# LiWentomng/OrientedRepPoints

Hardware: AMD Instinct MI355X
Metric: images/sec (1024x1024 DOTA, R-50 FPN) (higher is better)
Workload: dtype f32; 1 GPU; configs[1]: OrientedRepPoints R-50 FPN inference, 1024x1024 patch, 15 classes, bs=1/GPU, nms_pre=2000, score_thr=0.05, rnms iou_thr=0.4, max_per_img=2000; random-init weights, head biases calibrated to ~2000 dets/img; global_batch=1, parallelism=replicas x1 (image-parallel, no collective), images_in_flight_per_gpu=4

## Files before the change

include/orp_hip.h:

```cpp
#ifndef ORP_HIP_H_
#define ORP_HIP_H_

#include <stddef.h>
#include <stdint.h>

#ifdef __cplusplus
extern "C" {
#endif

#define ORP_OK 0
#define ORP_EINVAL (-1)
#define ORP_EWORKSPACE (-2)
#define ORP_ETOOBIG (-3)

const char* orp_version(void);

#define ORP_NMS_MAX_BOXES 131072
size_t orp_rnms_workspace_bytes(int n);
int orp_rnms(const float* dets, int n, float iou_thr, int flavor, int presorted, int order_out,
             int64_t* keep_out, int32_t* num_keep, void* workspace, size_t workspace_bytes, void* stream);

size_t orp_rnms_batched_workspace_bytes(int n_total, int nseg, int max_seg);
int orp_rnms_batched(const float* dets, int n_total, const int32_t* seg_offsets, int nseg, int max_seg,
                     float iou_thr, int flavor, int64_t* keep_out, int32_t* num_keep,
// ... 225 lines not shown
size_t orp_fpn_topdown_workspace_bytes(const orp_norm_level* levels, int nlevels, int batch, int channels, int groups);
int orp_fpn_topdown_nhwc(const orp_norm_level* levels, const float* const* gammas_host, const float* const* betas_host,
                         int nlevels, int batch, int channels, int groups, float eps, uint32_t* amax_out, void* workspace,
                         size_t workspace_bytes, void* stream);

typedef struct { const float* input; const float* residual; float* output; float* output2; int height; int width; } orp_bias_level;
int orp_bias_act_multi(const orp_bias_level* levels_host, int nlevels, int batch, int channels, const float* bias,
                       const float* sub, int relu, void* stream);

size_t orp_conv1x1_packed_floats(int c_in);
int orp_conv1x1_ok(int c_in, int c_out);
int orp_conv1x1_pack_weight(const float* weight, int c_out, int c_in, float* packed, void* stream);
int orp_conv1x1_multi(const orp_bias_level* levels_host, int nlevels, int batch, int c_in, int c_out,
                      const float* weight_packed, const float* bias, const float* sub, int relu, void* stream);

int orp_conv1x1_bn_act_ok(int c_in, int c_out);
int orp_conv1x1_bn_act_pays(int c_in, int c_out, int hw, int batch, int has_residual);
int orp_conv1x1_bn_act_tile(int c_in, int c_out, int hw, int batch, int* tile_channels, int* tile_positions);
int orp_conv1x1_bn_act(const float* x, const float* weight_t, const float* scale, const float* shift, const float* residual,
                       const float* scale2, const float* shift2, float* y, int batch, int c_in, int c_out, int hw, int relu,
                       void* stream);

int orp_conv1x1_bn_act_range(const float* x, const float* weight_t, const float* scale, const float* shift, const float* residual,
                             const float* scale2, const float* shift2, float* y, int batch, int c_in, int c_out, int hw, int relu,
                             uint32_t* range_out, void* stream);
int orp_conv1x1_bn_act_pieces_ok(int c_in, int c_out);
int orp_conv1x1_bn_act_pieces_pays(int c_in, int c_out, int hw, int batch, int has_residual);
int orp_conv1x1_bn_act_pieces_tile(int c_in, int c_out, int hw, int batch, int* tile_channels, int* tile_positions);
size_t orp_conv1x1_bn_pieces_packed_bytes(int c_in, int c_out);
int orp_conv1x1_bn_pieces_pack_weight(const float* weight, int c_in, int c_out, void* packed, void* stream);
int orp_conv1x1_bn_act_pieces(const float* x, const void* weight_packed, const float* scale, const float* shift,
                              const float* residual, const float* scale2, const float* shift2, float* y, int batch, int c_in,
                              int c_out, int hw, int relu, uint32_t* range_out, void* stream);

int orp_conv1x1_bn_act_pieces_dual_ok(int c_in, int c_in2, int c_out);
int orp_conv1x1_bn_act_pieces_dual_pays(int c_in, int c_in2, int c_out, int hw, int stride2, int batch);
int orp_conv1x1_bn_act_pieces_dual_tile(int c_in, int c_in2, int c_out, int hw, int batch, int* tile_channels, int* tile_positions);
int orp_conv1x1_bn_act_pieces_dual(const float* x, const void* w_packed, const float* scale, const float* shift, const float* x2,
                                   const void* w2_packed, const float* scale2, const float* shift2, int c_in2, int h2, int w2,
                                   int stride2, float* y, int batch, int c_in, int c_out, int ho, int wo, int relu, void* stream);

int orp_affine_act_range(const float* x, const float* residual, const float* scale, const float* shift, float* y, int batch,
                         int channels, int hw, int relu, uint32_t* range_out, void* stream);

int orp_conv3x3_bn_act_ok(int c_in, int c_out);
int orp_conv3x3_bn_act_pays(int c_in, int c_out, int height, int width, int batch);
int orp_conv3x3_bn_act_tile(int c_in, int c_out, int height, int width, int batch, int* tile_h, int* tile_w, int* waves_pos,
                            int* waves_ch);
size_t orp_conv3x3_bn_packed_bytes(int c_in, int c_out);
int orp_conv3x3_bn_pack_weight(const float* weight, int c_in, int c_out, void* packed, void* stream);
int orp_conv3x3_bn_act(const float* x, const void* weight_packed, const float* scale, const float* shift, const uint32_t* range_in,
                       float* y, int batch, int c_in, int c_out, int height, int width, int relu, void* stream);


int orp_conv3x3_small_ok(int c_in, int c_out);
int orp_conv3x3_small_multi(const orp_norm_level* levels_host, int nlevels, int batch, int c_in, int c_out,
                            const float* weight_packed, void* stream);
int orp_conv3x3_small_multi_ex(const orp_norm_level* levels_host, const float* const* weights_packed_host, int nlevels,
                               int batch, int c_in, int c_out, void* stream);
size_t orp_conv3x3_small_workspace_bytes(const orp_norm_level* levels_host, const int* strides_host, int nlevels, int batch,
                                         int c_out);
int orp_conv3x3_small_multi_strided(const orp_norm_level* levels_host, const float* const* weights_packed_host,
                                    const int* strides_host, int nlevels, int batch, int c_in, int c_out, void* workspace,
                                    size_t workspace_bytes, void* stream);

typedef struct { const float* input_a; const float* input_b; float* output_a; float* output_b; int height; int width; } orp_conv_level;
int orp_conv_split_ok(int c_in, int c_out, int kh, int kw);
int orp_conv_split_multi(const orp_conv_level* levels_host, int nlevels, int batch, int c_in, int c_out,
                         const float* weight_a_packed, const float* weight_b_packed, const float* bias_a, const float* bias_b,
                         int relu, int kh, int kw, int stride_h, int stride_w, int pad_h, int pad_w, int dil_h, int dil_w,
                         int out_layout, int nprod, void* workspace, size_t workspace_bytes, const uint32_t* amax_in,
                         int amax_stride, void* stream);
int orp_conv_split_multi_ex(const orp_conv_level* levels_host, const float* const* weights_packed_host,
                            const float* const* biases_host, int nlevels, int batch, int c_in, int c_out, int relu, int kh, int kw,
                            int stride_h, int stride_w, int pad_h, int pad_w, int dil_h, int dil_w, int out_layout, int nprod,
                            void* workspace, size_t workspace_bytes, const uint32_t* amax_in, void* stream);
size_t orp_conv_split_gn_partial_floats(const orp_conv_level* levels_host, int nlevels, int batch, int groups, int nlayers);
int orp_conv_split_multi_gn(const orp_conv_level* levels_host, int nlevels, int batch, int c_in, int c_out,
                            const float* weight_a_packed, const float* weight_b_packed, int kh, int kw, int pad_h, int pad_w,
                            int dil_h, int dil_w, int nprod, const float* coef_in, int relu_in, float* partials,
                            size_t partial_floats, int groups, void* workspace, size_t workspace_bytes, const uint32_t* amax_in,
                            int amax_stride, int amax_count, void* stream);
int orp_conv_split_gn_finish(const orp_conv_level* levels_host, int nlevels, int batch, int channels, int groups, int nlayers,
                             float eps, const float* const* gammas_host, const float* const* betas_host, const float* partials,
                             float* coef_out, uint32_t* bound_out, void* stream);
int orp_affine_act_multi_cl(const orp_norm_level* levels, int nlevels, int batch, int channels, const float* coef, int relu,
                            const uint32_t* bound_in, int nsets, int per_set, uint32_t* slot_out, void* stream);
int orp_conv_split_set_halo(int on);
int orp_conv_split_halo_tile(const orp_conv_level* levels_host, int nlevels, int batch, int c_in, int c_out, int kh, int kw, int stride,
                             int pad, int dil, int nprod, int* th, int* tw);
int orp_nchw_to_nhwc_multi(const orp_norm_level* levels_host, int nlevels, int batch, int channels, void* stream);
int orp_nchw_to_nhwc_multi_amax(const orp_norm_level* levels_host, int nlevels, int batch, int channels, const int* slots_host,
                                uint32_t* amax_out, int nslots, int reset, void* stream);

typedef struct { const float* input; const float* grad_output; int height; int width; } orp_wgrad_level;
int orp_conv_wgrad_split_ok(int c_in, int c_out, int kh, int kw);
size_t orp_conv_wgrad_split_workspace_bytes(const orp_wgrad_level* levels_host, int nlevels, int batch, int kh, int kw);
int orp_conv_wgrad_split(const orp_wgrad_level* levels_host, int nlevels, int batch, int c_in, int c_out, int kh, int kw,
                         int pad_h, int pad_w, int dil_h, int dil_w, const uint32_t* amax_x, const uint32_t* amax_g,
                         float* grad_weight, void* workspace, size_t workspace_bytes, void* stream);

int orp_window_attention(const float* qkv, const float* qkv_bias, const float* bias_table, int batch, int height, int width,
                         int heads, int head_dim, int window, int shift, float scale, float* out, void* stream);

int orp_window_attention_train(const float* qkv, const float* qkv_bias, const float* bias_table, int batch, int height, int width,
                               int heads, int head_dim, int window, int shift, float scale, float* out, float* lse, void* stream);
// ... 48 lines not shown
```

orientedreppoints_amd/_lib.py:

```python
import ctypes
import os

import torch

_HERE = os.path.dirname(os.path.abspath(__file__))
LIB_PATH = os.environ.get("ORP_HIP_LIB") or os.path.join(_HERE, "csrc", "liborp_hip.so")

ORP_OK, ORP_EINVAL, ORP_EWORKSPACE, ORP_ETOOBIG = 0, -1, -2, -3
ORP_NMS_MAX_BOXES = 131072

_vp = ctypes.c_void_p
_i = ctypes.c_int
_f = ctypes.c_float
_sz = ctypes.c_size_t

_SIGNATURES = {
    "orp_version": (ctypes.c_char_p, []),
    "orp_rnms_workspace_bytes": (_sz, [_i]),
    "orp_rnms": (_i, [_vp, _i, _f, _i, _i, _i, _vp, _vp, _vp, _sz, _vp]),
    "orp_rnms_batched_workspace_bytes": (_sz, [_i, _i, _i]),
    "orp_rnms_batched": (_i, [_vp, _i, _vp, _i, _i, _f, _i, _vp, _vp, _vp, _sz, _vp]),
    "_poly_nms": (None, [_vp, _vp, _vp, _i, _i, _f, _i]),
    "_overlaps": (None, [_vp, _vp, _vp, _i, _i, _i]),
    "orp_quad_iou_matrix": (_i, [_vp, _i, _vp, _i, _i, _i, _vp, _vp]),
# ... 43 lines not shown
    "orp_dcn_forward_h_tile_rows": (_i, [ctypes.c_long, _i]),
    "orp_dcn_forward_h_wave_specialised": (_i, []),
    "orp_dcn_forward_h_workspace_bytes": (_sz, [_vp, _i, _i, _i, _i]),
    "orp_dcn_forward_multi_h": (_i, [_vp, _vp, _i, _i, _i, _i, _vp, _vp] + [_i] * 12 + [_vp, _sz, _vp]),
    "orp_dcn_im2col": (_i, [_vp, _vp, _vp] + [_i] * 13 + [_vp, _vp]),
    "orp_dcn_col2im": (_i, [_vp, _vp, _vp, _vp] + [_i] * 13 + [_vp, _vp, _vp, _vp]),
    "orp_dcn_im2col_f64": (_i, [_vp, _vp, _vp] + [_i] * 13 + [_vp, _vp]),
    "orp_dcn_col2im_f64": (_i, [_vp, _vp, _vp, _vp] + [_i] * 13 + [_vp, _vp, _vp, _vp]),
    "orp_dcn_col2im_nhwc": (_i, [_vp, _vp, _vp] + [_i] * 12 + [_vp, _vp, _vp]),
    "orp_dcn_forward_direct": (_i, [_vp] * 6 + [_i] * 15 + [_vp]),
    "orp_dcn_backward_mfma_ok": (_i, [_i] * 6),
    "orp_dcn_backward_workspace_bytes": (_sz, [_vp] + [_i] * 10),
    "orp_dcn_backward_multi": (_i, [_vp, _i, _i, _i, _i, _vp, _vp] + [_i] * 9 + [_vp, _sz, _vp]),
    "orp_dcn_backward_multi_ex": (_i, [_vp, _vp, _vp, _i, _i, _i, _i, _i, _vp, _vp] + [_i] * 9 + [_vp, _sz, _vp]),
    "orp_poly_nms_f64_workspace_bytes": (_sz, [_i]),
    "orp_poly_nms_f64": (_i, [_vp, _i, ctypes.c_double, _vp, _vp, _vp, _sz, _vp]),
    "orp_poly_nms_f64_batched_workspace_bytes": (_sz, [_i, _i, _i]),
    "orp_poly_nms_f64_batched": (_i, [_vp, _i, _vp, _i, _i, ctypes.c_double, _i, _i, _vp, _vp, _vp, _sz, _vp]),
    "orp_scene_tiles": (_i, [_vp, _i, _i, ctypes.c_longlong, _vp, _i, _i, _vp, _vp, _i, _i, _vp, _vp]),
    "orp_scene_tiles_resized": (_i, [_vp, _i, _i, ctypes.c_longlong, _vp, _i, _i, _i, _i, _i, _i, _i, _vp, _vp, _vp, _vp, _vp, _vp, _i,
                                     _i, _vp, _vp]),
    "orp_scene_tiles_flip": (_i, [_vp, _i, _i, ctypes.c_longlong, _vp, _i, _i, _vp, _vp, _i, _i, _vp, _vp]),
    "orp_scene_tiles_resized_flip": (_i, [_vp, _i, _i, ctypes.c_longlong, _vp, _i, _i, _i, _i, _i, _i, _i, _vp, _vp, _vp, _vp, _vp,
                                          _vp, _i, _i, _vp, _vp]),
    "orp_scene_collect_workspace_bytes": (_sz, [_i, _i]),
    "orp_scene_collect": (_i, [_vp, _i, _i, _vp, ctypes.c_double, _i, _i, _vp, _vp, _vp, _vp, _vp, _sz, _vp]),
    "orp_soft_rnms_host": (_i, [_vp, _i, _f, _i, _f, _f, _vp, _vp]),
    "orp_conv1x1_packed_floats": (_sz, [_i]),
    "orp_conv1x1_ok": (_i, [_i, _i]),
    "orp_conv1x1_pack_weight": (_i, [_vp, _i, _i, _vp, _vp]),
    "orp_conv1x1_multi": (_i, [_vp, _i, _i, _i, _i, _vp, _vp, _vp, _i, _vp]),
    "orp_conv1x1_bn_act_ok": (_i, [_i, _i]),
    "orp_conv1x1_bn_act_pays": (_i, [_i, _i, _i, _i, _i]),
    "orp_conv1x1_bn_act_tile": (_i, [_i, _i, _i, _i, _vp, _vp]),
    "orp_conv1x1_bn_act": (_i, [_vp, _vp, _vp, _vp, _vp, _vp, _vp, _vp, _i, _i, _i, _i, _i, _vp]),
    "orp_conv1x1_bn_act_range": (_i, [_vp, _vp, _vp, _vp, _vp, _vp, _vp, _vp, _i, _i, _i, _i, _i, _vp, _vp]),
    "orp_affine_act_range": (_i, [_vp, _vp, _vp, _vp, _vp, _i, _i, _i, _i, _vp, _vp]),
    "orp_conv1x1_bn_act_pieces_ok": (_i, [_i, _i]),
    "orp_conv1x1_bn_act_pieces_pays": (_i, [_i, _i, _i, _i, _i]),
    "orp_conv1x1_bn_act_pieces_tile": (_i, [_i, _i, _i, _i, _vp, _vp]),
    "orp_conv1x1_bn_pieces_packed_bytes": (_sz, [_i, _i]),
    "orp_conv1x1_bn_pieces_pack_weight": (_i, [_vp, _i, _i, _vp, _vp]),
    "orp_conv1x1_bn_act_pieces": (_i, [_vp, _vp, _vp, _vp, _vp, _vp, _vp, _vp, _i, _i, _i, _i, _i, _vp, _vp]),
    "orp_conv1x1_bn_act_pieces_dual_ok": (_i, [_i, _i, _i]),
    "orp_conv1x1_bn_act_pieces_dual_pays": (_i, [_i, _i, _i, _i, _i, _i]),
    "orp_conv1x1_bn_act_pieces_dual_tile": (_i, [_i, _i, _i, _i, _i, _vp, _vp]),
    "orp_conv1x1_bn_act_pieces_dual": (_i, [_vp, _vp, _vp, _vp, _vp, _vp, _vp, _vp, _i, _i, _i, _i, _vp, _i, _i, _i, _i, _i, _i, _vp]),
    "orp_conv3x3_bn_act_ok": (_i, [_i, _i]),
    "orp_conv3x3_bn_act_pays": (_i, [_i, _i, _i, _i, _i]),
    "orp_conv3x3_bn_act_tile": (_i, [_i, _i, _i, _i, _i, _vp, _vp, _vp, _vp]),
    "orp_conv3x3_bn_packed_bytes": (_sz, [_i, _i]),
    "orp_conv3x3_bn_pack_weight": (_i, [_vp, _i, _i, _vp, _vp]),
    "orp_conv3x3_bn_act": (_i, [_vp, _vp, _vp, _vp, _vp, _vp, _i, _i, _i, _i, _i, _i, _vp]),
    "orp_pp_select_scratch_bytes": (_sz, [_i, _i, _i]),
    "orp_pp_select": (_i, [_vp, _i, _i, _vp, _i, _i, _vp, _vp, _sz, _vp]),
    "orp_pp_gather": (_i, [_vp, _vp, _i, _i, _vp, _vp, _vp, _i, _vp, _vp, _vp, _vp, _vp]),
    "orp_pp_compact_scratch_bytes": (_sz, [_i]),
    "orp_pp_compact": (_i, [_vp, _vp, _i, _i, _i, _vp, _f, _i, _vp, _vp, _vp, _vp, _vp, _vp, _sz, _vp]),
    "orp_pp_compact_views_scratch_bytes": (_sz, [_i]),
    "orp_pp_compact_views": (_i, [_vp, _i, _i, _f, _i, _vp, _vp, _vp, _vp, _vp, _vp, _vp, _vp, _sz, _vp]),
    "orp_pp_pack": (_i, [_vp, _vp, _vp, _vp, _vp, _vp, _vp, _vp, _i, _i, _vp, _vp]),
    "orp_groupnorm_workspace_bytes": (_sz, [_vp, _i, _i, _i, _i]),
    "orp_groupnorm_act_multi": (_i, [_vp, _i, _i, _i, _i, _vp, _vp, _f, _i, _vp, _sz, _vp]),
    "orp_groupnorm_act_multi_ex": (_i, [_vp, _vp, _vp, _i, _i, _i, _i, _f, _i, _vp, _sz, _vp]),
    "orp_groupnorm_act_multi_nhwc": (_i, [_vp, _vp, _vp, _vp, _i, _i, _i, _i, _f, _i, _vp, _sz, _vp]),
    "orp_groupnorm_act_multi_train": (_i, [_vp, _vp, _vp, _i, _i, _i, _i, _f, _i, _vp, _vp, _sz, _vp]),
    "orp_groupnorm_backward_workspace_bytes": (_sz, [_vp, _i, _i, _i, _i]),
    "orp_groupnorm_act_multi_backward": (_i, [_vp, _vp, _vp, _vp, _vp, _vp, _vp, _i, _i, _i, _i, _i, _vp, _vp, _sz, _vp]),
    "orp_voc_best_match_f64": (_i, [_vp, _vp, _i, _vp, _vp, _i, _vp, _vp, _vp]),
    "orp_affine_act": (_i, [_vp, _vp, _vp, _vp, _vp, _i, _i, _i, _i, _vp]),
    "orp_affine2_act": (_i, [_vp, _vp, _vp, _vp, _vp, _vp, _vp, _i, _i, _i, _i, _vp]),
    "orp_affine_relu_maxpool": (_i, [_vp, _vp, _vp, _vp, _i, _i, _i, _i, _vp]),
    "orp_fpn_topdown_workspace_bytes": (_sz, [_vp, _i, _i, _i, _i]),
    "orp_fpn_topdown_nhwc": (_i, [_vp, _vp, _vp, _i, _i, _i, _i, _f, _vp, _vp, _sz, _vp]),
    "orp_bias_act_multi": (_i, [_vp, _i, _i, _i, _vp, _vp, _i, _vp]),
    "orp_conv3x3_small_ok": (_i, [_i, _i]),
    "orp_conv3x3_small_multi": (_i, [_vp, _i, _i, _i, _i, _vp, _vp]),
    "orp_conv3x3_small_multi_ex": (_i, [_vp, _vp, _i, _i, _i, _i, _vp]),
    "orp_border_rows": (_i, [_vp, _vp, _vp, _i, _vp, _vp, _vp, _vp]),
    "orp_giou_rows": (_i, [_vp, _vp, _vp, _vp, _vp, _i, _f, _vp, _vp, _vp]),
    "orp_segment_finish": (_i, [_vp, _vp, _vp, _i, _i, _vp, _f, _i, _vp, _vp, _vp]),
    "orp_conv3x3_small_workspace_bytes": (ctypes.c_size_t, [_vp, _vp, _i, _i, _i]),
    "orp_conv3x3_small_multi_strided": (_i, [_vp, _vp, _vp, _i, _i, _i, _i, _vp, ctypes.c_size_t, _vp]),
    "orp_conv_split_ok": (_i, [_i, _i, _i, _i]),
    "orp_conv_split_multi": (_i, [_vp, _i, _i, _i, _i, _vp, _vp, _vp, _vp] + [_i] * 11 + [_vp, _sz, _vp, _i, _vp]),
    "orp_conv_split_multi_ex": (_i, [_vp, _vp, _vp, _i, _i, _i, _i] + [_i] * 11 + [_vp, _sz, _vp, _vp]),
    "orp_conv_split_set_halo": (_i, [_i]),
    "orp_conv_split_halo_tile": (_i, [_vp] + [_i] * 10 + [_vp, _vp]),
    "orp_conv_wgrad_split_ok": (_i, [_i, _i, _i, _i]),
    "orp_conv_wgrad_split_workspace_bytes": (_sz, [_vp, _i, _i, _i, _i]),
    "orp_conv_wgrad_split": (_i, [_vp, _i, _i, _i, _i, _i, _i, _i, _i, _i, _i, _vp, _vp, _vp, _vp, _sz, _vp]),
    "orp_nchw_to_nhwc_multi_amax": (_i, [_vp, _i, _i, _i, _vp, _vp, _i, _i, _vp]),
    "orp_groupnorm_act_multi_cl_amax": (_i, [_vp, _vp, _vp, _i, _i, _i, _i, _f, _i, _vp, _vp, _i, _vp, _sz, _vp]),
    "orp_dcn_forward_pair_amax": (_i, [_vp, _vp, _vp, _i, _i, _i, _i, _vp, _vp, _vp, _vp] + [_i] * 11 + [_vp, _sz, _vp, _i, _vp]),
    "orp_nchw_to_nhwc_multi": (_i, [_vp, _i, _i, _i, _vp]),
    "orp_groupnorm_cl_workspace_bytes": (_sz, [_vp, _i, _i, _i, _i]),
    "orp_groupnorm_act_multi_cl": (_i, [_vp, _vp, _vp, _i, _i, _i, _i, _f, _i, _vp, _sz, _vp]),
    "orp_debug_amax_log": (_i, [_vp, _i]),
    "orp_conv_split_gn_partial_floats": (_sz, [_vp, _i, _i, _i, _i]),
    "orp_conv_split_multi_gn": (_i, [_vp, _i, _i, _i, _i, _vp, _vp] + [_i] * 7 + [_vp, _i, _vp, _sz, _i, _vp, _sz, _vp, _i, _i, _vp]),
    "orp_conv_split_gn_finish": (_i, [_vp, _i, _i, _i, _i, _i, _f, _vp, _vp, _vp, _vp, _vp, _vp]),
    "orp_affine_act_multi_cl": (_i, [_vp, _i, _i, _i, _vp, _i, _vp, _i, _i, _vp, _vp]),
    "orp_window_attention": (_i, [_vp, _vp, _vp] + [_i] * 7 + [_f, _vp, _vp]),
    "orp_window_attention_train": (_i, [_vp, _vp, _vp] + [_i] * 7 + [_f, _vp, _vp, _vp]),
    "orp_window_attention_backward_workspace_bytes": (_sz, [_i] * 6),
    "orp_window_attention_backward": (_i, [_vp] * 6 + [_i] * 7 + [_f, _vp, _vp, _vp, _vp, _sz, _vp]),
# ... 74 lines not shown
```

orientedreppoints_amd/build.py:

```python
import concurrent.futures
import os
import subprocess

HERE = os.path.dirname(os.path.abspath(__file__))
CSRC = os.path.join(HERE, "csrc")
LIB = os.path.join(CSRC, "liborp_hip.so")
HIPCC = os.environ.get("HIPCC", "/opt/rocm/bin/hipcc")
ARCH = "gfx950"

NO_PACKED_FP32 = ["-Xclang", "-target-feature", "-Xclang", "-packed-fp32-ops"]
COMMON = ["--offload-arch=" + ARCH, "-O3", "-std=c++17", "-fPIC", "-Wall", "-Wno-unused-function",
          "-Wno-unused-result", "-Wno-unused-value",
          "-Wno-bitwise-instead-of-logical"]
if os.environ.get("ORP_PACKED_FP32", "0") != "1":
    COMMON = COMMON + NO_PACKED_FP32
SOURCES = [
    ("orp_nms.hip", ["-ffp-contract=off"]),
    ("orp_overlaps.hip", ["-ffp-contract=off"]),
    ("orp_minarearect.hip", ["-ffp-contract=off"]),
    ("orp_box_iou_rotated.hip", ["-ffp-contract=off"]),
    ("orp_convex.hip", ["-ffp-contract=off"]),
    ("orp_convex_giou.hip", ["-ffp-contract=off"]),
    ("orp_pointwise.hip", ["-ffp-contract=off"]),
    ("orp_assign.hip", ["-ffp-contract=off"]),
    ("orp_postproc.hip", ["-ffp-contract=off"]),
    ("orp_soft_rnms.hip", ["-ffp-contract=off"]),
    ("orp_scene.hip", ["-ffp-contract=off"]),
    ("orp_eval.hip", ["-ffp-contract=off"]),
    ("orp_train.hip", ["-ffp-contract=off"]),
    ("orp_norm.hip", []),
    ("orp_conv_small.hip", []),
    ("orp_conv1x1.hip", []),
    ("orp_conv1x1_bn.hip", []),
    ("orp_conv1x1_bn_pieces.hip", []),
    ("orp_conv3x3_bn.hip", []),
    ("orp_dcn.hip", []),
    ("orp_dcn_split.hip", ["-ffp-contract=off"]),
    ("orp_conv_split.hip", []),
    ("orp_conv_wgrad.hip", []),
    ("orp_dcn_half.hip", []),
    ("orp_dcn_bwd.hip", []),
    ("orp_dcn_bwd_mfma.hip", []),
    ("orp_window_attn.hip", []),
    ("orp_prof.hip", []),
]
HEADERS = ["orp_affine.hpp", "orp_geom.hpp", "orp_quadfast.hpp", "orp_tile.hpp", "orp_hull.hpp", "orp_libm.hpp", "orp_prof.hpp", "orp_launch.hpp", "orp_dcn_split.hpp", "orp_dcn_common.hpp", "orp_range.hpp", "orp_conv1x1_bn_host.hpp", os.path.join("..", "..", "include", "orp_hip.h")]


def _stale(target, deps):
    if not os.path.exists(target):
        return True
    t = os.path.getmtime(target)
    return any(os.path.getmtime(d) > t for d in deps if os.path.exists(d))


VERSION_SOURCE = "orp_overlaps.hip"


def build_id():
    import hashlib
    h = hashlib.sha1()
    names = sorted([s for s, _ in SOURCES] + [x for x in HEADERS])
    for n in names:
        path = os.path.join(CSRC, n)
        if os.path.exists(path):
            h.update(n.encode())
            h.update(open(path, "rb").read())
    return h.hexdigest()[:12]


def _compile(src, extra):
    obj = os.path.join(CSRC, os.path.splitext(src)[0] + ".o")
    deps = [os.path.join(CSRC, src)] + [os.path.join(CSRC, h) for h in HEADERS] + [os.path.abspath(__file__)]
    if src == VERSION_SOURCE:
        deps += [os.path.join(CSRC, s) for s, _ in SOURCES]
        extra = extra + ['-DORP_BUILD_ID="%s"' % build_id()]
    if _stale(obj, deps):
        cmd = [HIPCC] + COMMON + extra + ["-c", os.path.join(CSRC, src), "-o", obj]
        r = subprocess.run(cmd, cwd=CSRC, stderr=subprocess.PIPE, universal_newlines=True)
        err = "\n".join(l for l in r.stderr.splitlines() if "'-packed-fp32-ops' is not a recognized feature" not in l)
        if err.strip():
            import sys
            sys.stderr.write(err + "\n")
        if r.returncode != 0:
            raise subprocess.CalledProcessError(r.returncode, cmd)
    return obj


# ... 22 lines not shown
```

orientedreppoints_amd/mmdet_models/resnet.py:

```python
import torch
import torch.nn as nn

from .. import switches
from .layers import build_conv_layer, build_norm_layer, constant_init, kaiming_init
from .registry import BACKBONES


class Bottleneck(nn.Module):
    expansion = 4

    def __init__(self, inplanes, planes, stride=1, dilation=1, downsample=None, style='pytorch',
                 norm_cfg=dict(type='BN'), dcn=None):
        super(Bottleneck, self).__init__()
        assert style in ['pytorch', 'caffe']
        assert dcn is None or isinstance(dcn, dict)
        if style == 'pytorch':
            conv1_stride, conv2_stride = 1, stride
        else:
            conv1_stride, conv2_stride = stride, 1
        self.conv1 = nn.Conv2d(inplanes, planes, kernel_size=1, stride=conv1_stride, bias=False)
        self.add_module('bn1', build_norm_layer(norm_cfg, planes)[1])
        self.with_dcn = dcn is not None
        fallback_on_stride = False
        if self.with_dcn:
            fallback_on_stride = dcn.pop('fallback_on_stride', False)
            dcn = dict(dcn)
            if 'modulated' in dcn:
                dcn.setdefault('type', 'DCNv2' if dcn.pop('modulated') else 'DCN')
            dcn.setdefault('type', 'DCN')
        use_dcn = self.with_dcn and not fallback_on_stride
        self.conv2 = build_conv_layer(dcn if use_dcn else None, planes, planes, kernel_size=3, stride=conv2_stride,
                                      padding=dilation, dilation=dilation, bias=False)
        self.conv2_is_dcn = use_dcn
        self.add_module('bn2', build_norm_layer(norm_cfg, planes)[1])
        self.conv3 = nn.Conv2d(planes, planes * self.expansion, kernel_size=1, bias=False)
        self.add_module('bn3', build_norm_layer(norm_cfg, planes * self.expansion)[1])
        self.relu = nn.ReLU(inplace=True)
        self.downsample = downsample

    def _fused_ok(self, x):
        return (not torch.is_grad_enabled()) and x.is_cuda and x.dtype == torch.float32 and \
            isinstance(self.bn1, nn.BatchNorm2d) and not self.bn1.training and not self.bn3.training

    def _downsample_norm_fusable(self):
        return switches.of(self, 'fuse_downsample_norm', 'BN_DOWNSAMPLE_FUSE') and self._downsample_is_conv_norm()

    def _downsample_is_conv_norm(self):
        ds = self.downsample
        return isinstance(ds, nn.Sequential) and len(ds) == 2 and isinstance(ds[0], nn.Conv2d) and \
            isinstance(ds[1], nn.BatchNorm2d) and not ds[1].training

    def _conv1x1_fusable(self):
        return switches.of(self, 'fuse_conv1x1', 'BN_CONV1X1_FUSE')

    def _conv1x1_pieces_on(self):
        return switches.of(self, 'fuse_conv1x1_pieces', 'BN_CONV1X1_PIECES')

    def _downsample_conv_fusable(self):
        return switches.of(self, 'fuse_downsample_conv', 'BN_DOWNSAMPLE_CONV_FUSE')

    def _conv3x3_fusable(self):
        return switches.of(self, 'fuse_conv3x3', 'BN_CONV3X3_FUSE') and not self.conv2_is_dcn and \
            isinstance(self.bn2, nn.BatchNorm2d) and not self.bn2.training

    def _forward_fused(self, x):
        from ..mmdet_ops.fused_norm import bn_act, conv1x1_bn_act, conv3x3_bn_act, conv3x3_bn_act_routed, \
            conv1x1_bn_act_dual, conv1x1_bn_act_dual_routed
        fuse = self._conv1x1_fusable()
        pieces = None if self._conv1x1_pieces_on() else False

        def conv_bn_act(t, conv, bn, **kw):
            if fuse:
                return conv1x1_bn_act(t, conv, bn, pieces=pieces, **kw)
            return bn_act(conv(t).contiguous(), bn, **kw)
        force3 = bool(getattr(self, 'force_conv3x3', False))
        fuse3 = False
        if self._conv3x3_fusable() and tuple(self.conv1.stride) == (1, 1):
            fuse3 = conv3x3_bn_act_routed(x, self.conv2, self.bn2, force3,
                                          shape=(x.size(0), self.conv1.out_channels, x.size(2), x.size(3)))
        if fuse3:
            out, bits = conv_bn_act(x, self.conv1, self.bn1, relu=True, want_range=True)
            out = conv3x3_bn_act(out, self.conv2, self.bn2, relu=True, force=force3, range_bits=bits)
        else:
            out = conv_bn_act(x, self.conv1, self.bn1, relu=True)
            out = bn_act(self.conv2(out).contiguous(), self.bn2, relu=True)
        ds = self.downsample
        if fuse and pieces is None and self._downsample_conv_fusable() and self._downsample_is_conv_norm() and \
                conv1x1_bn_act_dual_routed(out, self.conv3, self.bn3, x, ds[0], ds[1]):
            return conv1x1_bn_act_dual(out, self.conv3, self.bn3, x, ds[0], ds[1], relu=True)
        if self._downsample_norm_fusable():
            residual, residual_bn = ds[0](x).contiguous(), ds[1]
        elif ds is not None:
            residual, residual_bn = bn_act(ds[0](x).contiguous(), ds[1], relu=False), None
        else:
            residual, residual_bn = x.contiguous(), None
        return conv_bn_act(out, self.conv3, self.bn3, residual=residual, residual_bn=residual_bn, relu=True)

    def forward(self, x):
        if self._fused_ok(x):
            return self._forward_fused(x)
        identity = x
        out = self.relu(self.bn1(self.conv1(x)))
        out = self.relu(self.bn2(self.conv2(out)))
        out = self.bn3(self.conv3(out))
        if self.downsample is not None:
            identity = self.downsample(x)
        out += identity
        return self.relu(out)


@BACKBONES.register_module
class ResNet(nn.Module):
    arch_settings = {50: (Bottleneck, (3, 4, 6, 3)), 101: (Bottleneck, (3, 4, 23, 3)), 152: (Bottleneck, (3, 8, 36, 3))}

    def __init__(self, depth, in_channels=3, num_stages=4, strides=(1, 2, 2, 2), dilations=(1, 1, 1, 1),
                 out_indices=(0, 1, 2, 3), style='pytorch', frozen_stages=-1, conv_cfg=None,
                 norm_cfg=dict(type='BN', requires_grad=True), norm_eval=True, dcn=None,
                 stage_with_dcn=(False, False, False, False), gcb=None, stage_with_gcb=None, gen_attention=None,
                 stage_with_gen_attention=None, with_cp=False, zero_init_residual=True):
        super(ResNet, self).__init__()
        if depth not in self.arch_settings:
            raise KeyError('invalid depth {} for resnet'.format(depth))
        assert gcb is None and gen_attention is None, 'context / attention blocks are not part of the DOTA configs'
        assert conv_cfg is None, 'the backbone convolutions are stock nn.Conv2d (dcn= selects the deformable conv2)'
        self.dcn = dict(dcn) if dcn is not None else None
        self.stage_with_dcn = tuple(stage_with_dcn) if stage_with_dcn is not None else (False,) * num_stages
        if dcn is not None:
            assert len(self.stage_with_dcn) == num_stages
        self.depth, self.num_stages, self.out_indices = depth, num_stages, out_indices
        self.frozen_stages, self.norm_eval = frozen_stages, norm_eval
        self.zero_init_residual = zero_init_residual
        block, stage_blocks = self.arch_settings[depth]
        self.conv1 = nn.Conv2d(in_channels, 64, kernel_size=7, stride=2, padding=3, bias=False)
        self.add_module('bn1', build_norm_layer(norm_cfg, 64)[1])
        self.relu = nn.ReLU(inplace=True)
# ... 101 lines not shown
```

orientedreppoints_amd/mmdet_ops/fused_norm.py:

```python
import ctypes

import torch

from .. import _lib, _packcache


class _NormLevel(ctypes.Structure):
    _fields_ = [("input", ctypes.c_void_p), ("output", ctypes.c_void_p), ("height", ctypes.c_int),
                ("width", ctypes.c_int)]


def _call(name, device, *args):
    with torch.cuda.device(device):
        rc = getattr(_lib.lib(), name)(*args)
    _lib.check(rc, name)


def _norm_levels(ins, outs):
    levels = (_NormLevel * len(ins))()
    for i, (x, y) in enumerate(zip(ins, outs)):
        levels[i] = _NormLevel(x.data_ptr(), y.data_ptr() if y is not None else None, x.size(2), x.size(3))
    return levels


# ... 270 lines not shown
    if not conv1x1_bn_act_dual_ok(x, conv, bn, x2, conv2, bn2):
        raise ValueError("conv1x1_bn_act_dual: unsupported modules or shapes (conv1x1_bn_act_dual_ok)")
    x, x2 = x.detach().contiguous(), x2.detach().contiguous()
    B, cin, H, W = x.shape
    cout, cin2 = conv.weight.size(0), conv2.weight.size(1)
    packed, packed2 = _packed_1x1_planes(conv.weight), _packed_1x1_planes(conv2.weight)
    scale, shift = _bn_affine(bn)
    scale2, shift2 = _bn_affine(bn2)
    y = torch.empty((B, cout, H, W), dtype=torch.float32, device=x.device)
    _call("orp_conv1x1_bn_act_pieces_dual", x.device, _lib.ptr(x), _lib.ptr(packed), _lib.ptr(scale), _lib.ptr(shift), _lib.ptr(x2),
          _lib.ptr(packed2), _lib.ptr(scale2), _lib.ptr(shift2), cin2, x2.size(2), x2.size(3), conv2.stride[0], _lib.ptr(y),
          B, cin, cout, H, W, 1 if relu else 0, _lib.stream_of(x))
    return y


def conv3x3_bn_act_ok(x, conv, bn, shape=None):
    w = getattr(conv, 'weight', None)
    shape = tuple(x.shape) if shape is None else tuple(shape)
    return bool(type(conv) is torch.nn.Conv2d and _bn_input(x, bn) and len(shape) == 4 and
                _plain_conv(conv, w, 3, ((1, 1),), 1) and shape[1] == w.size(1) and shape[0] * shape[2] * shape[3] > 0 and
                _lib.lib().orp_conv3x3_bn_act_ok(w.size(1), w.size(0)))


def conv3x3_bn_act_routed(x, conv, bn, force=False, shape=None):
    if not conv3x3_bn_act_ok(x, conv, bn, shape):
        return False
    B, _c, H, W = tuple(x.shape) if shape is None else tuple(shape)
    return bool(force or _lib.lib().orp_conv3x3_bn_act_pays(conv.weight.size(1), conv.weight.size(0), H, W, B))


def conv3x3_bn_act_tile(cin, cout, H, W, B):
    return _tile_query("orp_conv3x3_bn_act_tile", 4, cin, cout, H, W, B)


_packed_3x3 = _packcache.new_cache("conv3x3_bn_weight")


def _packed_3x3_planes(weight):
    return _packed_planes(_packed_3x3, weight, "orp_conv3x3_bn_packed_bytes", "orp_conv3x3_bn_pack_weight",
                          lambda w: w.float().contiguous())


def conv3x3_bn_act(x, conv, bn, relu=True, force=False, range_bits=None):
    if range_bits is None or not conv3x3_bn_act_routed(x, conv, bn, force):
        return bn_act(conv(x).contiguous(), bn, relu=relu)
    x = x.detach().contiguous()
    B, cin, H, W = x.shape
    cout = conv.weight.size(0)
    packed = _packed_3x3_planes(conv.weight)
    scale, shift = _bn_affine(bn)
    y = torch.empty((B, cout, H, W), dtype=torch.float32, device=x.device)
    _call("orp_conv3x3_bn_act", x.device, _lib.ptr(x), _lib.ptr(packed), _lib.ptr(scale), _lib.ptr(shift), _lib.ptr(range_bits),
          _lib.ptr(y), B, cin, cout, H, W, 1 if relu else 0, _lib.stream_of(x))
    return y


def bn_relu_maxpool(x, bn):
    if not (x.is_cuda and x.dtype == torch.float32 and x.dim() == 4 and x.is_contiguous()):
        raise ValueError("bn_relu_maxpool expects a contiguous fp32 CUDA [B,C,H,W] tensor")
    scale, shift = _bn_affine(bn)
    B, C, H, W = x.shape
    y = torch.empty((B, C, (H - 1) // 2 + 1, (W - 1) // 2 + 1), dtype=torch.float32, device=x.device)
    _call("orp_affine_relu_maxpool", x.device, _lib.ptr(x), _lib.ptr(scale), _lib.ptr(shift), _lib.ptr(y), B, C, H, W, _lib.stream_of(x))
    return y


def fpn_topdown_ok(xs, gns):
    x0, g0 = xs[0], gns[0]
    B, C = x0.size(0), x0.size(1)
    if not (1 <= len(xs) <= 4 and len(gns) == len(xs) and C % 32 == 0 and C % g0.num_groups == 0 and 32 % (C // g0.num_groups) == 0):
        return False
    for i, (x, g) in enumerate(zip(xs, gns)):
        if not (x.is_cuda and x.dtype == torch.float32 and x.dim() == 4 and x.size(0) == B and x.size(1) == C and
                isinstance(g, torch.nn.GroupNorm) and g.affine and g.num_groups == g0.num_groups and g.eps == g0.eps):
            return False
        if i and (xs[i - 1].size(2) != 2 * x.size(2) or xs[i - 1].size(3) != 2 * x.size(3)):
            return False
    return True


def fpn_topdown_cl(xs, gns, amax=True):
    if not fpn_topdown_ok(xs, gns):
        raise ValueError("fpn_topdown_cl: see fpn_topdown_ok")
    L = _lib.lib()
    x0 = xs[0]
    B, C = x0.size(0), x0.size(1)
    n = len(xs)
    gns, mods, owner = _gn_modules(gns, n, "fpn_topdown_cl")
    ins = [x.detach().contiguous() for x in xs]
    outs = [torch.empty(x.shape, dtype=torch.float32, device=x.device, memory_format=torch.channels_last) for x in ins]
    levels = _norm_levels(ins, outs)
    gam, bet, _gs, _bs = _affine_ptrs(mods, owner)
    bits = torch.empty(1, dtype=torch.int32, device=x0.device) if (amax and _ranges_wanted()) else None
    nbytes = L.orp_fpn_topdown_workspace_bytes(levels, n, B, C, gns[0].num_groups)
    ws = _lib.workspace(x0.device, nbytes)
    _call("orp_fpn_topdown_nhwc", x0.device, levels, gam, bet, n, B, C, gns[0].num_groups, float(gns[0].eps),
          bits.data_ptr() if bits is not None else None, _lib.ptr(ws), ws.numel(), _lib.stream_of(x0))
    return outs, bits


class _BiasLevel(ctypes.Structure):
    _fields_ = [("input", ctypes.c_void_p), ("residual", ctypes.c_void_p), ("output", ctypes.c_void_p),
                ("output2", ctypes.c_void_p), ("height", ctypes.c_int), ("width", ctypes.c_int)]


def bias_act_multi(xs, bias, relu=False, residuals=None, sub=None):
# ... 567 lines not shown
```

orientedreppoints_amd/switches.py:

```python
import os


def _on(name, default='1'):
    return os.environ.get(name, default) == '1'


TOWER_SPLIT = _on('ORP_TOWER_SPLIT')
FPN_SPLIT = _on('ORP_FPN_SPLIT')
TOWER_GN_FUSE = _on('ORP_TOWER_GN_FUSE')
BN_DOWNSAMPLE_FUSE = _on('ORP_BN_DOWNSAMPLE_FUSE')
BN_CONV1X1_FUSE = _on('ORP_BN_CONV1X1_FUSE')
BN_CONV1X1_PIECES = _on('ORP_BN_CONV1X1_PIECES')
BN_DOWNSAMPLE_CONV_FUSE = _on('ORP_BN_DOWNSAMPLE_CONV_FUSE')
BN_CONV3X3_FUSE = _on('ORP_BN_CONV3X3_FUSE')
STEM_POOL_FUSE = _on('ORP_STEM_POOL_FUSE')
SWIN_ATTN_FUSE = _on('ORP_SWIN_ATTN_FUSE')
SWIN_ATTN_TRAIN_FUSE = _on('ORP_SWIN_ATTN_TRAIN_FUSE')
SWIN_ATTN_HALF_FUSE = _on('ORP_SWIN_ATTN_HALF_FUSE')
FPN_TOPDOWN_FUSE = _on('ORP_FPN_TOPDOWN_FUSE')
TRAIN_SPLIT = _on('ORP_TRAIN_SPLIT')
DETERMINISTIC = _on('ORP_DETERMINISTIC', '0')


def of(obj, attr, name):
    on = getattr(obj, attr, None)
    return bool(globals()[name] if on is None else on)
```

Baseline: 428.0 images/s.

## Add fused deep-channel 3x3 conv+BN kernel using split-fp16 MFMA for layer4

Adds a HIP kernel for 512-in/512-out 3x3 convolutions with stride 1 or 2 that folds the BN affine and ReLU into the epilogue. It stages the input halo in LDS as hi/lo fp16 planes and uses three 32x32x16 f16 MFMAs per step to emulate fp32 accuracy, with a split-K reduction across waves. The ResNet bottleneck routes layer4's conv2 to this kernel when the shape table says it pays. The goal is to replace the separate conv and BN passes in the deepest stage; the cost is a custom code path with split-precision arithmetic and a fixed 512-channel specialization.

```diff
diff --git a/include/orp_hip.h b/include/orp_hip.h
--- a/include/orp_hip.h
+++ b/include/orp_hip.h
@@ -301,6 +301,13 @@
 int orp_conv3x3_bn_act(const float* x, const void* weight_packed, const float* scale, const float* shift, const uint32_t* range_in,
                        float* y, int batch, int c_in, int c_out, int height, int width, int relu, void* stream);
 
+int orp_conv3x3_bn_deep_ok(int c_in, int c_out, int stride);
+int orp_conv3x3_bn_deep_pays(int c_in, int c_out, int height, int width, int stride, int batch);
+size_t orp_conv3x3_bn_deep_packed_bytes(int c_in, int c_out);
+int orp_conv3x3_bn_deep_pack_weight(const float* weight, int c_in, int c_out, void* packed, void* stream);
+int orp_conv3x3_bn_deep(const float* x, const void* weight_packed, const float* scale, const float* shift, const uint32_t* range_in,
+                        float* y, int batch, int c_in, int c_out, int height, int width, int stride, int relu, void* stream);
+
 
 int orp_conv3x3_small_ok(int c_in, int c_out);
 int orp_conv3x3_small_multi(const orp_norm_level* levels_host, int nlevels, int batch, int c_in, int c_out,
diff --git a/orientedreppoints_amd/_lib.py b/orientedreppoints_amd/_lib.py
--- a/orientedreppoints_amd/_lib.py
+++ b/orientedreppoints_amd/_lib.py
@@ -119,6 +119,11 @@
     "orp_conv3x3_bn_packed_bytes": (_sz, [_i, _i]),
     "orp_conv3x3_bn_pack_weight": (_i, [_vp, _i, _i, _vp, _vp]),
     "orp_conv3x3_bn_act": (_i, [_vp, _vp, _vp, _vp, _vp, _vp, _i, _i, _i, _i, _i, _i, _vp]),
+    "orp_conv3x3_bn_deep_ok": (_i, [_i, _i, _i]),
+    "orp_conv3x3_bn_deep_pays": (_i, [_i, _i, _i, _i, _i, _i]),
+    "orp_conv3x3_bn_deep_packed_bytes": (_sz, [_i, _i]),
+    "orp_conv3x3_bn_deep_pack_weight": (_i, [_vp, _i, _i, _vp, _vp]),
+    "orp_conv3x3_bn_deep": (_i, [_vp, _vp, _vp, _vp, _vp, _vp, _i, _i, _i, _i, _i, _i, _i, _vp]),
     "orp_pp_select_scratch_bytes": (_sz, [_i, _i, _i]),
     "orp_pp_select": (_i, [_vp, _i, _i, _vp, _i, _i, _vp, _vp, _sz, _vp]),
     "orp_pp_gather": (_i, [_vp, _vp, _i, _i, _vp, _vp, _vp, _i, _vp, _vp, _vp, _vp, _vp]),
diff --git a/orientedreppoints_amd/build.py b/orientedreppoints_amd/build.py
--- a/orientedreppoints_amd/build.py
+++ b/orientedreppoints_amd/build.py
@@ -34,6 +34,7 @@
     ("orp_conv1x1_bn.hip", []),
     ("orp_conv1x1_bn_pieces.hip", []),
     ("orp_conv3x3_bn.hip", []),
+    ("orp_conv3x3_bn_deep.hip", []),
     ("orp_dcn.hip", []),
     ("orp_dcn_split.hip", ["-ffp-contract=off"]),
     ("orp_conv_split.hip", []),
diff --git a/orientedreppoints_amd/csrc/orp_conv3x3_bn_deep.hip b/orientedreppoints_amd/csrc/orp_conv3x3_bn_deep.hip
--- /dev/null
+++ b/orientedreppoints_amd/csrc/orp_conv3x3_bn_deep.hip
@@ -0,0 +1,263 @@
+#include <hip/hip_runtime.h>
+#include <stdint.h>
+
+#include "../../include/orp_hip.h"
+#include "orp_affine.hpp"
+#include "orp_range.hpp"
+#include "orp_launch.hpp"
+#include "orp_dcn_split.hpp"
+
+namespace {
+
+typedef float floatx16 __attribute__((ext_vector_type(16)));
+typedef _Float16 h8 __attribute__((ext_vector_type(8)));
+typedef _Float16 h2 __attribute__((ext_vector_type(2)));
+
+constexpr int kThreads = 512;
+constexpr int C = 512;
+constexpr int TH = 2, TW = 16;
+constexpr int NCH = 4;
+
+struct Args {
+  const float* x;
+  const uint16_t* planes;
+  size_t plane_stride;
+  const float* wscale;
+  const unsigned* range;
+  const float* scale; const float* shift;
+  float* y;
+  int H, W, Ho, Wo, relu, tiles_x, tiles_per_image;
+};
+
+template <int S, int KS>
+struct Cfg {
+  static constexpr int WN = 8 / KS;
+  static constexpr int CG = 32 * WN;
+  static constexpr int KH = C / KS;
+  static constexpr int HROWS = (TH - 1) * S + 3, HCOLS = (TW - 1) * S + 3;
+  static constexpr int ROWS = HROWS * HCOLS;
+  static constexpr int CST = S == 1 ? C : 128;
+  static constexpr int NPASS = C / CST;
+  static constexpr int PB = CST / KS / 64;
+  static constexpr int PPH = 9 * PB;
+  static constexpr int ASTR = CST + 8;
+  static constexpr size_t smem = (size_t)2 * ROWS * ASTR * 2;
+  static_assert(smem <= 163840, "a workgroup may take 160 KiB of LDS");
+  static_assert(PB >= 1 && smem >= (size_t)(KS - 1) * WN * 16 * 64 * sizeof(float), "the reduction reuses the halo's area");
+  static __device__ __forceinline__ int row(int hy, int hx) { return S == 1 ? hy * HCOLS + hx : hy * HCOLS + (hx & 1) * 17 + (hx >> 1); }
+};
+
+template <int S, int KS>
+__global__ void __launch_bounds__(kThreads)
+conv3x3_bn_deep_kernel(const Args P) {
+  using K = Cfg<S, KS>;
+  constexpr int CG = K::CG, KH = K::KH;
+  constexpr int ASTR = K::ASTR, PLANE = K::ROWS * ASTR, HCOLS = K::HCOLS;
+  extern __shared__ __attribute__((aligned(16))) unsigned char smem[];
+  uint16_t* sA = reinterpret_cast<uint16_t*>(smem);
+
+  const int tid = threadIdx.x, lane = tid & 63, wave = tid >> 6;
+  const int cgrp = blockIdx.x % (C / CG), tile = blockIdx.x / (C / CG);
+  const int img = tile / P.tiles_per_image, tt = tile - img * P.tiles_per_image;
+  const int trow = tt / P.tiles_x;
+  const int y0 = trow * TH, x0 = (tt - trow * P.tiles_x) * TW;
+  const int H = P.H, W = P.W;
+  const size_t hw = (size_t)H * W;
+
+  const int kx = orp::range_exp(*P.range);
+  const float sx = orp::range_scale(kx);
+  const int kxw = kx + orp::range_exp_of(*P.wscale);
+
+  const int wn = wave % K::WN, g = wave / K::WN;
+  const int n_wave = cgrp * CG + wn * 32;
+  const int mrow = lane & 31, kg = lane >> 5;
+  const uint16_t* wp = P.planes + ((size_t)kg * C + n_wave + mrow) * 8;
+  constexpr size_t wblk = (size_t)2 * C * 8;
+  auto load_b = [&](int q, int j, h8 (&b)[2]) {
+    const int pass = q / K::PPH, ph = q - pass * K::PPH;
+    const int tap = ph / K::PB, cb = ph - tap * K::PB;
+    const uint16_t* a = wp + (size_t)(tap * (C / 16) + (g * KH + pass * (K::CST / KS) + cb * 64) / 16 + j) * wblk;
+#pragma unroll
+    for (int pl = 0; pl < 2; pl++) b[pl] = *reinterpret_cast<const h8*>(a + (size_t)pl * P.plane_stride);
+  };
+  h8 bq[NCH][2];
+#pragma unroll
+  for (int j = 0; j < NCH; j++) load_b(0, j, bq[j]);
+  __builtin_amdgcn_sched_barrier(0);
+
+  const int ty = mrow >> 4, tx = (mrow - 2 * ty) & 15;
+  const uint16_t* abase = sA + (size_t)K::row(S * ty, 0) * ASTR + (size_t)tx * ASTR + g * (K::CST / KS) + 8 * kg;
+  auto a_off = [&](int ph) {
+    const int tap = ph / K::PB, cb = ph - tap * K::PB;
+    const int ki = tap / 3, kj = tap - 3 * ki;
+    return K::row(ki, kj) * ASTR + cb * 64;
+  };
+  auto load_a = [&](int off, int j, h8 (&a)[2]) {
+#pragma unroll
+    for (int pl = 0; pl < 2; pl++) a[pl] = *reinterpret_cast<const h8*>(abase + pl * PLANE + off + j * 16);
+  };
+
+  floatx16 acc = floatx16{0}, side = floatx16{0};
+  constexpr int nphase = K::NPASS * K::PPH;
+
+#pragma unroll 1
+  for (int pass = 0; pass < K::NPASS; pass++) {
+    if (pass > 0) __syncthreads();
+    {
+      const int px = lane & 15, cq = lane >> 4;
+      const float* xb = P.x + ((size_t)img * C + (size_t)pass * (K::CST / KS) + (size_t)((wave * 4 + cq) * 2)) * hw;
+      constexpr int NPB = (K::ROWS + 15) / 16, NCB = K::CST / 64;
+      constexpr int G = S == 1 ? 5 : 11;
+      static_assert(G >= NPB, "one batch of loads per pass");
+      float v[G][NCB][2];
+      bool in[G];
+#pragma unroll
+      for (int gi = 0; gi < G; gi++) {
+        const int h = gi * 16 + px;
+        const int hy = h / HCOLS, hx = h - hy * HCOLS;
+        const int yy = S * y0 - 1 + hy, xx = S * x0 - 1 + hx;
+        in[gi] = h < K::ROWS && yy >= 0 && yy < H && xx >= 0 && xx < W;
+        const float* src = xb + (in[gi] ? (size_t)yy * W + xx : (size_t)0);
+#pragma unroll
+        for (int cb = 0; cb < NCB; cb++) {
+          const int ch = (cb / K::PB) * KH + (cb % K::PB) * 64;
+          v[gi][cb][0] = src[(size_t)ch * hw];
+          v[gi][cb][1] = src[(size_t)(ch + 1) * hw];
+        }
+      }
+#pragma unroll
+      for (int gi = 0; gi < G; gi++)
+#pragma unroll
+        for (int cb = 0; cb < NCB; cb++) { asm volatile("" : "+v"(v[gi][cb][0])); asm volatile("" : "+v"(v[gi][cb][1])); }
+#pragma unroll
+      for (int gi = 0; gi < G; gi++) {
+        const int h = gi * 16 + px;
+        const int hy = h / HCOLS, hx = h - hy * HCOLS;
+#pragma unroll
+        for (int cb = 0; cb < NCB; cb++) {
+          const float s0 = in[gi] ? v[gi][cb][0] * sx : 0.f, s1 = in[gi] ? v[gi][cb][1] * sx : 0.f;
+          h2 hh, ll;
+          orp::range_split(s0, hh, ll, 0);
+          orp::range_split(s1, hh, ll, 1);
+          if (h < K::ROWS) {
+            uint16_t* dst = sA + (size_t)K::row(hy, hx) * ASTR + cb * 64 + (wave * 4 + cq) * 2;
+            *reinterpret_cast<unsigned*>(dst) = __builtin_bit_cast(unsigned, hh);
+            *reinterpret_cast<unsigned*>(dst + PLANE) = __builtin_bit_cast(unsigned, ll);
+          }
+        }
+      }
+    }
+    __syncthreads();
+
+    h8 a[2][2];
+    load_a(a_off(0), 0, a[0]);
+#pragma unroll 1
+    for (int ph = 0; ph < K::PPH; ph++) {
+      const int q = pass * K::PPH + ph;
+      const int q_n = q + 1 < nphase ? q + 1 : q;
+      const int off = a_off(ph), off_n = a_off(ph + 1 < K::PPH ? ph + 1 : ph);
+#pragma unroll
+      for (int j = 0; j < NCH; j++) {
+        if (j + 1 < NCH) load_a(off, j + 1, a[(j + 1) & 1]);
+        else             load_a(off_n, 0, a[0]);
+        __builtin_amdgcn_sched_barrier(0);
+        side = __builtin_amdgcn_mfma_f32_32x32x16_f16(bq[j][0], a[j & 1][1], side, 0, 0, 0);
+        side = __builtin_amdgcn_mfma_f32_32x32x16_f16(bq[j][1], a[j & 1][0], side, 0, 0, 0);
+        acc = __builtin_amdgcn_mfma_f32_32x32x16_f16(bq[j][0], a[j & 1][0], acc, 0, 0, 0);
+        __builtin_amdgcn_sched_barrier(0);
+        load_b(q_n, j, bq[j]);
+        __builtin_amdgcn_sched_barrier(0);
+      }
+    }
+  }
+
+  float* red = reinterpret_cast<float*>(smem) + (size_t)wn * 16 * 64 + lane;
+  constexpr int RG = K::WN * 16 * 64;
+  __syncthreads();
+  if (g > 0) {
+#pragma unroll
+    for (int r = 0; r < 16; r++) red[(g - 1) * RG + r * 64] = acc[r] + side[r];
+  }
+  __syncthreads();
+  if (g > 0) return;
+
+  const int yy = y0 + ty, xx = x0 + tx;
+  if (yy < P.Ho && xx < P.Wo) {
+    const size_t hwo = (size_t)P.Ho * P.Wo;
+    float* o = P.y + (size_t)img * C * hwo + (size_t)yy * P.Wo + xx;
+#pragma unroll
+    for (int r = 0; r < 16; r++) {
+      const int ch = n_wave + (r & 3) + 8 * (r >> 2) + 4 * kg;
+      float t = acc[r] + side[r];
+#pragma unroll
+      for (int k = 0; k < KS - 1; k++) t += red[k * RG + r * 64];
+      const float v = orp::range_unscale(t, kxw);
+      o[(size_t)ch * hwo] = affine_act(v, P.scale[ch], P.shift[ch], P.relu);
+    }
+  }
+}
+
+template <int S, int KS>
+hipError_t launch(const Args& A, long tiles, hipStream_t st) {
+  using K = Cfg<S, KS>;
+  struct Tag {};
+  hipError_t e = orp::set_max_dynamic_lds_once<Tag>(reinterpret_cast<const void*>(&conv3x3_bn_deep_kernel<S, KS>), K::smem);
+  if (e != hipSuccess) return e;
+  hipLaunchKernelGGL((conv3x3_bn_deep_kernel<S, KS>), dim3((unsigned)(tiles * (C / K::CG))), dim3(kThreads), K::smem, st, A);
+  return hipGetLastError();
+}
+
+}
+
+extern "C" {
+
+int orp_conv3x3_bn_deep_ok(int c_in, int c_out, int stride) {
+  return (c_in == C && c_out == C && (stride == 1 || stride == 2)) ? 1 : 0;
+}
+
+size_t orp_conv3x3_bn_deep_packed_bytes(int c_in, int c_out) {
+  return orp_conv3x3_bn_deep_ok(c_in, c_out, 1) ? (size_t)4 * c_in * c_out * 9 + 16 : 0;
+}
+
+int orp_conv3x3_bn_deep_pack_weight(const float* weight, int c_in, int c_out, void* packed, void* stream) {
+  if (!weight || !packed || ((uintptr_t)packed & 15) || !orp_conv3x3_bn_deep_ok(c_in, c_out, 1)) return ORP_EINVAL;
+  uint16_t* planes = reinterpret_cast<uint16_t*>(packed);
+  const size_t n = (size_t)c_in * c_out * 9;
+  hipError_t e = orp_split::pack_planes16(weight, c_out, c_in, 9, planes, reinterpret_cast<float*>(planes + 2 * n), (hipStream_t)stream);
+  return e == hipSuccess ? ORP_OK : (int)e;
+}
+
+int orp_conv3x3_bn_deep_pays(int c_in, int c_out, int height, int width, int stride, int batch) {
+  if (!orp_conv3x3_bn_deep_ok(c_in, c_out, stride) || height <= 0 || width <= 0 || batch <= 0) return 0;
+  static const struct { int stride, side_min, side_max, batch; } paid[] = {
+      {1, 32, 48, 1}, {1, 32, 32, 2},
+      {2, 64, 96, 1}, {2, 64, 64, 2},
+  };
+  for (const auto& s : paid)
+    if (s.stride == stride && s.batch == batch && height >= s.side_min && height <= s.side_max && width >= s.side_min && width <= s.side_max)
+      return 1;
+  return 0;
+}
+
+int orp_conv3x3_bn_deep(const float* x, const void* weight_packed, const float* scale, const float* shift, const uint32_t* range_in,
+                        float* y, int batch, int c_in, int c_out, int height, int width, int stride, int relu, void* stream) {
+  if (!x || !weight_packed || ((uintptr_t)weight_packed & 15) || !scale || !shift || !range_in || !y || (const float*)y == x || batch <= 0 ||
+      height <= 0 || width <= 0 || !orp_conv3x3_bn_deep_ok(c_in, c_out, stride))
+    return ORP_EINVAL;
+  Args A;
+  A.x = x; A.scale = scale; A.shift = shift; A.y = y; A.range = range_in;
+  A.planes = reinterpret_cast<const uint16_t*>(weight_packed);
+  A.plane_stride = (size_t)c_out * c_in * 9;
+  A.wscale = reinterpret_cast<const float*>(A.planes + 2 * A.plane_stride);
+  A.H = height; A.W = width; A.relu = relu ? 1 : 0;
+  A.Ho = (height - 1) / stride + 1; A.Wo = (width - 1) / stride + 1;
+  A.tiles_x = (A.Wo + TW - 1) / TW;
+  const long tpi = (long)A.tiles_x * ((A.Ho + TH - 1) / TH);
+  if (tpi * batch * 8 >= (1L << 31) || (long)height * width >= (1L << 31)) return ORP_ETOOBIG;
+  A.tiles_per_image = (int)tpi;
+  hipStream_t st = (hipStream_t)stream;
+  hipError_t e = stride == 1 ? launch<1, 4>(A, tpi * batch, st) : launch<2, 2>(A, tpi * batch, st);
+  return e == hipSuccess ? ORP_OK : (int)e;
+}
+
+}
diff --git a/orientedreppoints_amd/mmdet_models/resnet.py b/orientedreppoints_amd/mmdet_models/resnet.py
--- a/orientedreppoints_amd/mmdet_models/resnet.py
+++ b/orientedreppoints_amd/mmdet_models/resnet.py
@@ -63,9 +63,13 @@
         return switches.of(self, 'fuse_conv3x3', 'BN_CONV3X3_FUSE') and not self.conv2_is_dcn and \
             isinstance(self.bn2, nn.BatchNorm2d) and not self.bn2.training
 
+    def _conv3x3_deep_fusable(self):
+        return switches.of(self, 'fuse_conv3x3_deep', 'BN_CONV3X3_DEEP_FUSE') and not self.conv2_is_dcn and \
+            isinstance(self.bn2, nn.BatchNorm2d) and not self.bn2.training
+
     def _forward_fused(self, x):
         from ..mmdet_ops.fused_norm import bn_act, conv1x1_bn_act, conv3x3_bn_act, conv3x3_bn_act_routed, \
-            conv1x1_bn_act_dual, conv1x1_bn_act_dual_routed
+            conv3x3_bn_deep, conv3x3_bn_deep_routed, conv1x1_bn_act_dual, conv1x1_bn_act_dual_routed
         fuse = self._conv1x1_fusable()
         pieces = None if self._conv1x1_pieces_on() else False
 
@@ -78,9 +82,17 @@
         if self._conv3x3_fusable() and tuple(self.conv1.stride) == (1, 1):
             fuse3 = conv3x3_bn_act_routed(x, self.conv2, self.bn2, force3,
                                           shape=(x.size(0), self.conv1.out_channels, x.size(2), x.size(3)))
+        force3d = bool(getattr(self, 'force_conv3x3_deep', False))
+        deep3 = False
+        if not fuse3 and self._conv3x3_deep_fusable() and tuple(self.conv1.stride) == (1, 1):
+            deep3 = conv3x3_bn_deep_routed(x, self.conv2, self.bn2, force3d,
+                                           shape=(x.size(0), self.conv1.out_channels, x.size(2), x.size(3)))
         if fuse3:
             out, bits = conv_bn_act(x, self.conv1, self.bn1, relu=True, want_range=True)
             out = conv3x3_bn_act(out, self.conv2, self.bn2, relu=True, force=force3, range_bits=bits)
+        elif deep3:
+            out, bits = conv_bn_act(x, self.conv1, self.bn1, relu=True, want_range=True)
+            out = conv3x3_bn_deep(out, self.conv2, self.bn2, relu=True, force=force3d, range_bits=bits)
         else:
             out = conv_bn_act(x, self.conv1, self.bn1, relu=True)
             out = bn_act(self.conv2(out).contiguous(), self.bn2, relu=True)
diff --git a/orientedreppoints_amd/mmdet_ops/fused_norm.py b/orientedreppoints_amd/mmdet_ops/fused_norm.py
--- a/orientedreppoints_amd/mmdet_ops/fused_norm.py
+++ b/orientedreppoints_amd/mmdet_ops/fused_norm.py
@@ -346,6 +346,43 @@
     y = torch.empty((B, cout, H, W), dtype=torch.float32, device=x.device)
     _call("orp_conv3x3_bn_act", x.device, _lib.ptr(x), _lib.ptr(packed), _lib.ptr(scale), _lib.ptr(shift), _lib.ptr(range_bits),
           _lib.ptr(y), B, cin, cout, H, W, 1 if relu else 0, _lib.stream_of(x))
+    return y
+
+
+def conv3x3_bn_deep_ok(x, conv, bn, shape=None):
+    w = getattr(conv, 'weight', None)
+    shape = tuple(x.shape) if shape is None else tuple(shape)
+    return bool(type(conv) is torch.nn.Conv2d and _bn_input(x, bn) and len(shape) == 4 and
+                _plain_conv(conv, w, 3, ((1, 1), (2, 2)), 1) and shape[1] == w.size(1) and shape[0] * shape[2] * shape[3] > 0 and
+                _lib.lib().orp_conv3x3_bn_deep_ok(w.size(1), w.size(0), conv.stride[0]))
+
+
+def conv3x3_bn_deep_routed(x, conv, bn, force=False, shape=None):
+    if not conv3x3_bn_deep_ok(x, conv, bn, shape):
+        return False
+    B, _c, H, W = tuple(x.shape) if shape is None else tuple(shape)
+    return bool(force or _lib.lib().orp_conv3x3_bn_deep_pays(conv.weight.size(1), conv.weight.size(0), H, W, conv.stride[0], B))
+
+
+_packed_3x3_deep = _packcache.new_cache("conv3x3_bn_deep_weight")
+
+
+def _packed_3x3_deep_planes(weight):
+    return _packed_planes(_packed_3x3_deep, weight, "orp_conv3x3_bn_deep_packed_bytes", "orp_conv3x3_bn_deep_pack_weight",
+                          lambda w: w.float().contiguous())
+
+
+def conv3x3_bn_deep(x, conv, bn, relu=True, force=False, range_bits=None):
+    if range_bits is None or not conv3x3_bn_deep_routed(x, conv, bn, force):
+        return bn_act(conv(x).contiguous(), bn, relu=relu)
+    x = x.detach().contiguous()
+    B, cin, H, W = x.shape
+    cout, s = conv.weight.size(0), conv.stride[0]
+    packed = _packed_3x3_deep_planes(conv.weight)
+    scale, shift = _bn_affine(bn)
+    y = torch.empty((B, cout, (H - 1) // s + 1, (W - 1) // s + 1), dtype=torch.float32, device=x.device)
+    _call("orp_conv3x3_bn_deep", x.device, _lib.ptr(x), _lib.ptr(packed), _lib.ptr(scale), _lib.ptr(shift), _lib.ptr(range_bits),
+          _lib.ptr(y), B, cin, cout, H, W, s, 1 if relu else 0, _lib.stream_of(x))
     return y
 
 
diff --git a/orientedreppoints_amd/switches.py b/orientedreppoints_amd/switches.py
--- a/orientedreppoints_amd/switches.py
+++ b/orientedreppoints_amd/switches.py
@@ -13,6 +13,7 @@
 BN_CONV1X1_PIECES = _on('ORP_BN_CONV1X1_PIECES')
 BN_DOWNSAMPLE_CONV_FUSE = _on('ORP_BN_DOWNSAMPLE_CONV_FUSE')
 BN_CONV3X3_FUSE = _on('ORP_BN_CONV3X3_FUSE')
+BN_CONV3X3_DEEP_FUSE = _on('ORP_BN_CONV3X3_DEEP_FUSE')
 STEM_POOL_FUSE = _on('ORP_STEM_POOL_FUSE')
 SWIN_ATTN_FUSE = _on('ORP_SWIN_ATTN_FUSE')
 SWIN_ATTN_TRAIN_FUSE = _on('ORP_SWIN_ATTN_TRAIN_FUSE')
```

Result: faster. 442.0 images/s (median of 6 runs) (+3.3%).
